# 23skdu/longbow

Measured on AMD Instinct MI355X. Metric: k-NN queries/sec (batch=1024, k=100), 1Mx768 f32, higher is better.
Workload: dtype f32; 1 GPU; 1Mx768 float32 cosine, batch=1024 queries, k=100, brute-force; dim=768, batch=1024, k=100, metric=cosine, global_rows=1000000, candidate_mode=LB_CAND_F32_MFMA (strict; the library default is AUTO: auto_path leg)

## Files before the change

### longbow_amd/_lib.py

```python
import ctypes as C
import os

_HERE = os.path.dirname(os.path.abspath(__file__))
SO_PATH = os.environ.get("LB_GPU_SO") or os.path.join(_HERE, "liblongbow_gpu.so")

LB_OK = 0
STATUS = {0: "ok", 1: "invalid argument", 2: "index is closed", 3: "GPU not available",
          4: "HIP runtime error", 5: "out of device memory", 6: "unsupported configuration",
          7: "internal error", 8: "context canceled", 9: "context deadline exceeded"}


class LongbowGPUError(RuntimeError):
    def __init__(self, code, msg=""):
        self.code = code
        super().__init__(f"longbow_gpu: {STATUS.get(code, 'error')} (code {code}){': ' + msg if msg else ''}")


class GPUNotAvailable(LongbowGPUError):
    """internal/gpu/stub.go:10 ErrGPUNotAvailable"""


class Canceled(LongbowGPUError):
    """context.Canceled: the call's Cancel fired (internal/store/adaptive_index.go:182 returns ctx.Err())"""

# ... 229 lines not shown
    ("lb_gpu_ivfpq_dims", _i, [_vp]),
    ("lb_gpu_ivfpq_m", _i, [_vp]),
    ("lb_gpu_ivfpq_order", _i, [_vp]),
    ("lb_gpu_ivfpq_nlist", _i, [_vp]),
    ("lb_gpu_ivfpq_ntotal", _i64, [_vp]),
    ("lb_gpu_ivfpq_hbm_bytes", _i64, [_vp]),
    ("lb_gpu_ivfpq_get_centroids", _i, [_vp, _vp]),
    ("lb_gpu_ivfpq_reserve", _i, [_vp, _i64]),
    ("lb_gpu_ivfpq_add", _i, [_vp, _i64, _vp, _vp]),
    ("lb_gpu_ivfpq_add_device", _i, [_vp, _i64, _vp, _vp]),
    ("lb_gpu_ivfpq_get_codes", _i, [_vp, _i64, _i64, _vp]),
    ("lb_gpu_ivfpq_list_sizes", _i, [_vp, _vp]),
    ("lb_gpu_ivfpq_assignments", _i, [_vp, _i64, _i64, _vp]),
    ("lb_gpu_ivfpq_search", _i, [_vp, _i64, _vp, _i, _i, _vp, _vp]),
    ("lb_gpu_ivfpq_search_ctx", _i, [_vp, _i64, _vp, _i, _i, _vp, _vp, _vp]),
    ("lb_gpu_ivfpq_search_device_ctx", _i, [_vp, _i64, _vp, _i, _i, _vp, _vp, _vp, _vp]),
    ("lb_gpu_ivfpq_set_filter", _i, [_vp, _vp, _i64]),
    ("lb_gpu_ivfpq_filter_int64", _i, [_vp, _vp, _i64, _i64, _i, _vp, _i64, _i]),
    ("lb_gpu_ivfpq_filter_float32", _i, [_vp, _vp, _i64, C.c_float, _i, _vp, _i64, _i]),
    ("lb_gpu_ivfpq_nvisible", _i64, [_vp]),
    ("lb_gpu_ivfpq_last_search_stats", _i, [_vp, C.POINTER(C.c_int64)]),
    ("lb_gpu_ivfpq_set_profiling", _i, [_vp, _i]),
    ("lb_gpu_ivfpq_last_timing", _i, [_vp, _vp]),
    ("lb_gpu_ivfpq_last_build_timing", _i, [_vp, _vp]),
    ("lb_gpu_ivfpq_remove", _i, [_vp, _i64, _vp, C.POINTER(C.c_int64)]),
    ("lb_gpu_ivfpq_remove_device", _i, [_vp, _i64, _vp, C.POINTER(C.c_int64)]),
    ("lb_gpu_ivfpq_remove_rows", _i, [_vp, _i64, _vp, C.POINTER(C.c_int64)]),
    ("lb_gpu_ivfpq_nlive", _i64, [_vp]),
    ("lb_gpu_ivfpq_ndeleted", _i64, [_vp]),
    ("lb_gpu_ivfpq_compact", _i, [_vp, _vp, _i64]),
    ("lb_gpu_ivfsq8_new", _vp, [_i, _i, _vp, _vp, _i, _i, _vp, _ip]),
    ("lb_gpu_ivfsq8_free", None, [_vp]),
    ("lb_gpu_ivfsq8_last_error", C.c_char_p, [_vp]),
    ("lb_gpu_ivfsq8_dims", _i, [_vp]),
    ("lb_gpu_ivfsq8_order", _i, [_vp]),
    ("lb_gpu_ivfsq8_nlist", _i, [_vp]),
    ("lb_gpu_ivfsq8_ntotal", _i64, [_vp]),
    ("lb_gpu_ivfsq8_hbm_bytes", _i64, [_vp]),
    ("lb_gpu_ivfsq8_get_bounds", _i, [_vp, _vp, _vp]),
    ("lb_gpu_ivfsq8_get_centroids", _i, [_vp, _vp]),
    ("lb_gpu_ivfsq8_reserve", _i, [_vp, _i64]),
    ("lb_gpu_ivfsq8_add", _i, [_vp, _i64, _vp, _vp]),
    ("lb_gpu_ivfsq8_add_device", _i, [_vp, _i64, _vp, _vp]),
    ("lb_gpu_ivfsq8_get_codes", _i, [_vp, _i64, _i64, _vp]),
    ("lb_gpu_ivfsq8_list_sizes", _i, [_vp, _vp]),
    ("lb_gpu_ivfsq8_assignments", _i, [_vp, _i64, _i64, _vp]),
    ("lb_gpu_ivfsq8_search", _i, [_vp, _i64, _vp, _i, _i, _vp, _vp]),
    ("lb_gpu_ivfsq8_search_ctx", _i, [_vp, _i64, _vp, _i, _i, _vp, _vp, _vp]),
    ("lb_gpu_ivfsq8_search_device_ctx", _i, [_vp, _i64, _vp, _i, _i, _vp, _vp, _vp, _vp]),
    ("lb_gpu_ivfsq8_set_filter", _i, [_vp, _vp, _i64]),
    ("lb_gpu_ivfsq8_filter_int64", _i, [_vp, _vp, _i64, _i64, _i, _vp, _i64, _i]),
    ("lb_gpu_ivfsq8_filter_float32", _i, [_vp, _vp, _i64, C.c_float, _i, _vp, _i64, _i]),
    ("lb_gpu_ivfsq8_nvisible", _i64, [_vp]),
    ("lb_gpu_ivfsq8_last_search_stats", _i, [_vp, C.POINTER(C.c_int64)]),
    ("lb_gpu_ivfsq8_set_profiling", _i, [_vp, _i]),
    ("lb_gpu_ivfsq8_last_timing", _i, [_vp, _vp]),
    ("lb_gpu_ivfsq8_last_build_timing", _i, [_vp, _vp]),
    ("lb_gpu_ivfsq8_remove", _i, [_vp, _i64, _vp, C.POINTER(C.c_int64)]),
    ("lb_gpu_ivfsq8_remove_device", _i, [_vp, _i64, _vp, C.POINTER(C.c_int64)]),
    ("lb_gpu_ivfsq8_remove_rows", _i, [_vp, _i64, _vp, C.POINTER(C.c_int64)]),
    ("lb_gpu_ivfsq8_nlive", _i64, [_vp]),
    ("lb_gpu_ivfsq8_ndeleted", _i64, [_vp]),
    ("lb_gpu_ivfsq8_compact", _i, [_vp, _vp, _i64]),
    ("lb_gpu_ivfbq_new", _vp, [_i, _i, _i, _i, _vp, _ip]),
    ("lb_gpu_ivfbq_free", None, [_vp]),
    ("lb_gpu_ivfbq_last_error", C.c_char_p, [_vp]),
    ("lb_gpu_ivfbq_dims", _i, [_vp]),
    ("lb_gpu_ivfbq_words", _i, [_vp]),
    ("lb_gpu_ivfbq_order", _i, [_vp]),
    ("lb_gpu_ivfbq_nlist", _i, [_vp]),
    ("lb_gpu_ivfbq_ntotal", _i64, [_vp]),
    ("lb_gpu_ivfbq_hbm_bytes", _i64, [_vp]),
    ("lb_gpu_ivfbq_get_centroids", _i, [_vp, _vp]),
    ("lb_gpu_ivfbq_reserve", _i, [_vp, _i64]),
    ("lb_gpu_ivfbq_add", _i, [_vp, _i64, _vp, _vp]),
    ("lb_gpu_ivfbq_add_device", _i, [_vp, _i64, _vp, _vp]),
    ("lb_gpu_ivfbq_get_codes", _i, [_vp, _i64, _i64, _vp]),
    ("lb_gpu_ivfbq_list_sizes", _i, [_vp, _vp]),
    ("lb_gpu_ivfbq_assignments", _i, [_vp, _i64, _i64, _vp]),
    ("lb_gpu_ivfbq_search", _i, [_vp, _i64, _vp, _i, _i, _vp, _vp]),
    ("lb_gpu_ivfbq_search_ctx", _i, [_vp, _i64, _vp, _i, _i, _vp, _vp, _vp]),
    ("lb_gpu_ivfbq_search_device_ctx", _i, [_vp, _i64, _vp, _i, _i, _vp, _vp, _vp, _vp]),
    ("lb_gpu_ivfbq_set_filter", _i, [_vp, _vp, _i64]),
    ("lb_gpu_ivfbq_filter_int64", _i, [_vp, _vp, _i64, _i64, _i, _vp, _i64, _i]),
    ("lb_gpu_ivfbq_filter_float32", _i, [_vp, _vp, _i64, C.c_float, _i, _vp, _i64, _i]),
    ("lb_gpu_ivfbq_nvisible", _i64, [_vp]),
    ("lb_gpu_ivfbq_last_search_stats", _i, [_vp, C.POINTER(C.c_int64)]),
    ("lb_gpu_ivfbq_set_profiling", _i, [_vp, _i]),
    ("lb_gpu_ivfbq_last_timing", _i, [_vp, _vp]),
    ("lb_gpu_ivfbq_last_build_timing", _i, [_vp, _vp]),
    ("lb_gpu_merge_topk_device", _i, [_i, _i, _i64, _i, _vp, _vp, _vp, _vp, _vp]),
    ("lb_gpu_merge_topk_packed_device", _i, [_i, _i, _i64, _i, _vp, _vp, _vp, _vp]),
    ("lb_gpu_rrf_fuse_device", _i, [_i, _i64, _i, _vp, _i, _vp, _i, _i, _vp, _vp, _vp]),
    ("lb_gpu_rrf_fuse", _i, [_i, _i64, _i, _vp, _i, _vp, _i, _i, _vp, _vp]),
    ("lb_gpu_fill_uniform_device", _i, [_i, _vp, _i64, _u64, _i64, _vp]),
    ("lb_gpu_fill_codes_device", _i, [_i, _vp, _i64, _u64, _i64, _vp]),
    ("lb_gpu_fill_uniform_rows_device", _i, [_i, _vp, _vp, _i64, _i, _u64, _vp]),
    ("lb_gpu_shader_clock_mhz", C.c_double, [_i, _i]),
    ("lb_flight_datasets_new", _vp, []),
    ("lb_flight_datasets_free", None, [_vp]),
    ("lb_flight_datasets_put", _i, [_vp, C.c_char_p, _vp]),
    ("lb_flight_vector_search_exchange", _i, [_vp, _vp, _sz, C.POINTER(_vp), C.POINTER(_sz), C.c_char_p, _sz]),
    ("lb_flight_encode_results", _i, [_vp, _vp, _i64, C.POINTER(_vp), C.POINTER(_sz)]),
    ("lb_flight_free_buffer", None, [_vp]),
    ("lb_flight_index_add_ipc", _i, [_vp, _vp, _sz, C.POINTER(_i64), C.c_char_p, _sz]),
    ("lb_gpu_comm_init_all", _vp, [_i, _vp, _ip]),
    ("lb_gpu_comm_get_unique_id", _i, [_vp]),
    ("lb_gpu_comm_init_rank", _vp, [_i, _i, _i, _vp, _ip]),
    ("lb_gpu_comm_init_host", _vp, [_i, _i, _i, _vp, _vp, _ip]),
    ("lb_gpu_comm_free", None, [_vp]),
    ("lb_gpu_comm_prepare", _i, [_vp, _i64, _i]),
    ("lb_gpu_comm_nranks", _i, [_vp]),
    ("lb_gpu_comm_rank", _i, [_vp]),
    ("lb_gpu_comm_last_error", C.c_char_p, [_vp]),
    ("lb_gpu_comm_search_device", _i, [_vp, _vp, _i64, _vp, _i, _vp, _vp, _vp]),
    ("lb_gpu_comm_search_all", _i, [_vp, _vp, _i64, _vp, _i, _vp, _vp]),
    ("lb_gpu_index_set_profiling", _i, [_vp, _i]),
    ("lb_gpu_index_last_timing", _i, [_vp, _vp, _vp]),
]


def _bind(path, extra=()):
    if not os.path.exists(path):
        raise RuntimeError(
            f"{path} is missing: build it with `python -m longbow_amd.build{' --diag' if extra else ''}` "
            "(hipcc --offload-arch=gfx950).  There is no CPU fallback.")
    lib = C.CDLL(path)
    for name, res, args in list(SIGNATURES) + list(extra):
        fn = getattr(lib, name)
        fn.restype = res
        fn.argtypes = args
    return lib


def load():
    global _lib
    if _lib is None:
        _lib = _bind(SO_PATH)
    return _lib


DIAG_SO_PATH = os.path.join(_HERE, "liblongbow_gpu_diag.so")
DIAG_SIGNATURES = [
    ("lb_debug_set_sample_tau", None, [_i]),
    ("lb_debug_vmm_fail_next", None, [_i]),
    ("lb_debug_fused_fail_next", None, [_i]),
    ("lb_debug_tin_withhold_next", None, [_i]),
    ("lb_debug_search_fail_next", None, [_i]),
    ("lb_debug_set_add_register_min", None, [C.c_longlong]),
    ("lb_debug_sample_plan", None, [C.c_longlong, _i, C.c_uint, C.c_uint, C.POINTER(C.c_longlong)]),
    ("lb_debug_cand_geometry", None, [_i, C.POINTER(C.c_int), C.POINTER(C.c_uint)]),
    ("lb_debug_last_wide_rows", _i, []),
    ("lb_debug_set_wide256_min_tiles", None, [_i]),
    ("lb_debug_set_compact_round_rows", None, [C.c_longlong]),
]
_diag = None


def load_diag():
    global _diag
    if _diag is None:
        _diag = _bind(DIAG_SO_PATH, DIAG_SIGNATURES)
    return _diag


def require_gpu(device=0):
    lib = load()
    n = lib.lb_gpu_device_count()
    if n <= 0 or device >= n:
        raise GPUNotAvailable(3, f"{n} HIP device(s) visible, device {device} requested")
    return lib


def check(rc, handle=None, lib=None, prefix=None):
    if rc == LB_OK:
        return
    msg = ""
    if handle:
        lib = lib or load()
        raw = getattr(lib, prefix + "_last_error" if prefix else "lb_gpu_last_error")(handle)
        msg = raw.decode() if raw else ""
    if rc == 3:
        raise GPUNotAvailable(rc, msg)
    if rc == 8:
        raise Canceled(rc, msg)
    if rc == 9:
        raise DeadlineExceeded(rc, msg)
    raise LongbowGPUError(rc, msg)
```

### longbow_amd/csrc/kernels_gemm.hip

```cpp
#include "lb_admit.h"

#include <atomic>
#include <cstdlib>

namespace lb {

constexpr int BM = 128;
constexpr int BN = 128;
constexpr int BK = 32;
constexpr int GEMM_THREADS = 256;

struct GemmArgs {
    const float *X;
    const float *norm2;
    const float *rnorm;
    int64_t row_begin, row_end;
    int D;
    const float *Q;
    int nq;
    const uint8_t *mask;
    const uint32_t *rowmap;
    CandState cs;
    int n_row_tiles, n_q_tiles;
    int boot;
};

__device__ __forceinline__ int swz_off(int row, int chunk)
{
    return row * BK + ((chunk ^ ((row >> 1) & 7)) << 2);
}

template <int MODE>
__device__ __forceinline__ f32x4 load_chunk(const float *base, int64_t row, int D, int k)
{
    f32x4 v = {0.f, 0.f, 0.f, 0.f};
    const float *p = base + row * (int64_t)D + k;
    if (MODE == 2) {
        v = *reinterpret_cast<const f32x4 *>(p);
    } else if (MODE == 1) {
        if (k < D) v = *reinterpret_cast<const f32x4 *>(p);
    } else {
        if (k + 0 < D) v.x = p[0];
        if (k + 1 < D) v.y = p[1];
        if (k + 2 < D) v.z = p[2];
        if (k + 3 < D) v.w = p[3];
    }
    return v;
}

template <int METRIC, int ALIGNED>
__global__ __launch_bounds__(GEMM_THREADS, 2) void gemm_filter_kernel(GemmArgs a)
{
    constexpr bool GLDS = ALIGNED == 2;
    const int b = blockIdx.x;
    const int xcd = b & 7;
    const int in_xcd = b >> 3;
    const int qt = in_xcd % a.n_q_tiles;
    const int rt = (in_xcd / a.n_q_tiles) * 8 + xcd;
    if (rt >= a.n_row_tiles) return;

    __shared__ __attribute__((aligned(16))) float lds_all[2 * 2 * BM * BK + BM + BM + BM / 4];
    float(*lds)[2][BM * BK] = reinterpret_cast<float(*)[2][BM * BK]>(lds_all);
    float *s_aux = lds_all + 2 * 2 * BM * BK;
    uint32_t *s_rowid = reinterpret_cast<uint32_t *>(s_aux + BM);
    uint8_t *s_vis = reinterpret_cast<uint8_t *>(s_rowid + BM);

    const int tid = threadIdx.x;
    const int lane = tid & 63;
    const int wave = tid >> 6;
    const int wr = wave >> 1, wc = wave & 1;
    const int l31 = lane & 31, h = lane >> 5;

    const int64_t row0 = a.row_begin + (int64_t)rt * BM;
    const int q0 = qt * BN;
    const int64_t last_row = a.row_end - 1;
    const int last_q = a.nq - 1;

    auto corpus_row = [&](int64_t pos) -> int64_t {
        if (pos > last_row) pos = last_row;
        return a.rowmap ? (int64_t)a.rowmap[pos] : pos;
    };
    const int64_t side_ri = corpus_row(row0 + (tid & (BM - 1)));

    int st_row[4], st_ch[4];
    int64_t st_xrow[4];
    int st_qrow[4];
#pragma unroll
    for (int i = 0; i < 4; i++) {
        int c = tid + GEMM_THREADS * i;
        st_row[i] = c >> 3;
        st_ch[i] = c & 7;
        st_xrow[i] = corpus_row(row0 + st_row[i]);
        int qr = q0 + st_row[i];
        st_qrow[i] = qr < last_q ? qr : last_q;
    }

    f32x16 acc[2][2];
#pragma unroll
    for (int i = 0; i < 2; i++)
#pragma unroll
        for (int j = 0; j < 2; j++)
#pragma unroll
            for (int r = 0; r < 16; r++) acc[i][j][r] = 0.f;

    const int nk = (a.D + BK - 1) / BK;
    f32x4 ra[4], rb[4];

    const float *gsrcA[4], *gsrcB[4];
    if (GLDS) {
#pragma unroll
        for (int i = 0; i < 4; i++) {
            const int j = wave * 4 + i;
            const int row = j * 8 + (lane >> 3);
            const int c = (lane & 7) ^ ((row >> 1) & 7);
            const int64_t xr = corpus_row(row0 + row);
            int qr = q0 + row;
            if (qr > last_q) qr = last_q;
            gsrcA[i] = a.X + xr * (int64_t)a.D + 4 * c;
            gsrcB[i] = a.Q + (int64_t)qr * a.D + 4 * c;
        }
    }
    const int wave_u = __builtin_amdgcn_readfirstlane(wave);
    auto glds_piece = [&](int p, int stage, int k0) {
        const int i = p >> 1;
        const int j = wave_u * 4 + i;
        if ((p & 1) == 0)
            __builtin_amdgcn_global_load_lds(
                (const __attribute__((address_space(1))) void *)(gsrcA[i] + k0),
                (__attribute__((address_space(3))) void *)(&lds[stage][0][j * 8 * BK]), 16, 0,
                2);
        else
            __builtin_amdgcn_global_load_lds(
                (const __attribute__((address_space(1))) void *)(gsrcB[i] + k0),
                (__attribute__((address_space(3))) void *)(&lds[stage][1][j * 8 * BK]), 16, 0, 0);
    };
    auto glds_stage = [&](int stage, int k0) {
#pragma unroll
        for (int p = 0; p < 8; p++) glds_piece(p, stage, k0);
    };
    if (GLDS) glds_stage(0, 0);
    const float aux_r = side_aux<METRIC>(a.norm2, a.rnorm, side_ri);
    uint8_t side_vis = 1;
    if (a.mask) side_vis = a.mask[side_ri];
    uint64_t tau_raw[2];
#pragma unroll
    for (int tn = 0; tn < 2; tn++) {
        const int qj = q0 + wc * 64 + tn * 32 + l31;
        tau_raw[tn] = lane_tau(a.cs.tau, qj, a.nq, a.boot);
    }
    if (tid < BM) {
        s_aux[tid] = aux_r;
        s_vis[tid] = (row0 + tid <= last_row && side_vis) ? (uint8_t)1 : (uint8_t)0;
        s_rowid[tid] = (uint32_t)side_ri;
    }
    float tau_key[2];
    uint32_t tau_row[2];
#pragma unroll
    for (int tn = 0; tn < 2; tn++) {
// ... 102 lines not shown
            const float *As = lds[cur][0];
            const float *Bs = lds[cur][1];
            f32x4 fa[2][2], fb[2][2];
#pragma unroll
            for (int t = 0; t < 2; t++) {
                fa[0][t] = *reinterpret_cast<const f32x4 *>(&As[swz_off(wr * 64 + t * 32 + l31, h)]);
                fb[0][t] = *reinterpret_cast<const f32x4 *>(&Bs[swz_off(wc * 64 + t * 32 + l31, h)]);
            }
#pragma unroll
            for (int s = 0; s < 4; s++) {
                const int cb = s & 1, nb = cb ^ 1;
                if (s < 3) {
                    const int ch = 2 * (s + 1) + h;
#pragma unroll
                    for (int t = 0; t < 2; t++) {
                        fa[nb][t] = *reinterpret_cast<const f32x4 *>(&As[swz_off(wr * 64 + t * 32 + l31, ch)]);
                        fb[nb][t] = *reinterpret_cast<const f32x4 *>(&Bs[swz_off(wc * 64 + t * 32 + l31, ch)]);
                    }
                }
#pragma unroll
                for (int e = 0; e < 4; e++)
#pragma unroll
                    for (int tm = 0; tm < 2; tm++)
#pragma unroll
                        for (int tn = 0; tn < 2; tn++)
                            acc[tm][tn] = __builtin_amdgcn_mfma_f32_32x32x2f32(fa[cb][tm][e], fb[cb][tn][e],
                                                                              acc[tm][tn], 0, 0, 0);
                if (s == 1 && has_next) {
                    const int nxt = cur ^ 1;
#pragma unroll
                    for (int i = 0; i < 4; i++) {
                        *reinterpret_cast<f32x4 *>(&lds[nxt][0][swz_off(st_row[i], st_ch[i])]) = ra[i];
                        *reinterpret_cast<f32x4 *>(&lds[nxt][1][swz_off(st_row[i], st_ch[i])]) = rb[i];
                    }
                }
            }
            __syncthreads();
        }
    }

    float aux[2][4][4];
    uint32_t rid[2][4][4];
    uint32_t vbits = 0;
#pragma unroll
    for (int tm = 0; tm < 2; tm++)
#pragma unroll
        for (int g = 0; g < 4; g++)
            vbits |= tile_rows4(s_aux, s_rowid, s_vis, wr * 64 + tm * 32 + 8 * g + 4 * h, aux[tm][g], rid[tm][g]) << (tm * 16 + g * 4);
#pragma unroll
    for (int tn = 0; tn < 2; tn++) {
        const int qj = q0 + wc * 64 + tn * 32 + l31;
        const bool qok = qj < a.nq;
        uint64_t *list = a.cs.lists + (size_t)(qok ? qj : 0) * a.cs.cap;
        if (a.boot) {
            if (qok) {
#pragma unroll
                for (int tm = 0; tm < 2; tm++)
#pragma unroll
                    for (int g = 0; g < 4; g++) {
                        const int64_t rbase = row0 + wr * 64 + tm * 32 + 8 * g + 4 * h;
                        uint64_t ent[4];
#pragma unroll
                        for (int e = 0; e < 4; e++)
                            ent[e] = ((vbits >> (tm * 16 + g * 4 + e)) & 1u) ? pack_entry(cand_key<METRIC>(acc[tm][tn][4 * g + e], aux[tm][g][e]), rid[tm][g][e]) : kEntryMax;
                        uint64_t *dst = list + (rbase - a.row_begin);
                        if (rbase + 3 < a.row_end) {
                            typedef unsigned long long u64x2 __attribute__((ext_vector_type(2)));
                            u64x2 v0 = {ent[0], ent[1]}, v1 = {ent[2], ent[3]};
                            *reinterpret_cast<u64x2 *>(dst) = v0;
                            *reinterpret_cast<u64x2 *>(dst + 2) = v1;
                        } else {
#pragma unroll
                            for (int e = 0; e < 4; e++)
                                if (rbase + e < a.row_end) dst[e] = ent[e];
                        }
                    }
            }
            continue;
        }
        uint32_t bits = 0;
#pragma unroll
        for (int tm = 0; tm < 2; tm++)
#pragma unroll
            for (int g = 0; g < 4; g++)
#pragma unroll
                for (int e = 0; e < 4; e++)
                    bits |= admit_exact(cand_key<METRIC>(acc[tm][tn][4 * g + e], aux[tm][g][e]), rid[tm][g][e], tau_key[tn], tau_row[tn]) << (tm * 16 + g * 4 + e);
        bits &= vbits;
        if (bits) {
            uint32_t pos = atomicAdd(&a.cs.cnt[qj], (uint32_t)__builtin_popcount(bits));
#pragma unroll
            for (int tm = 0; tm < 2; tm++)
#pragma unroll
                for (int g = 0; g < 4; g++)
#pragma unroll
                    for (int e = 0; e < 4; e++)
                        if (bits & (1u << (tm * 16 + g * 4 + e))) {
                            const uint32_t ri = rid[tm][g][e];
                            if (pos < a.cs.cap) list[pos] = pack_entry(cand_key<METRIC>(acc[tm][tn][4 * g + e], aux[tm][g][e]), ri);
                            pos++;
                        }
        }
    }
}

constexpr int WBM = 256;
constexpr int WBK = 16;
constexpr int WNST = 3;
constexpr int W_STAGE_F = (WBM + BN) * WBK;
constexpr int W_NI = 6;

__device__ __forceinline__ int wswz(int row, int chunk) { return row * WBK + ((chunk ^ ((row >> 2) & 3)) << 2); }

template <bool NT>
__device__ __forceinline__ void wide_dma16(const void *gsrc, uint32_t lds_addr)
{
    uint32_t save;
    if (NT)
        asm volatile("s_mov_b32 %0, m0\n\ts_mov_b32 m0, %2\n\ts_nop 0\n\tglobal_load_lds_dwordx4 %1, off nt\n\ts_mov_b32 m0, %0"
                     : "=&s"(save) : "v"(gsrc), "s"(lds_addr) : "memory");
    else
        asm volatile("s_mov_b32 %0, m0\n\ts_mov_b32 m0, %2\n\ts_nop 0\n\tglobal_load_lds_dwordx4 %1, off\n\ts_mov_b32 m0, %0"
                     : "=&s"(save) : "v"(gsrc), "s"(lds_addr) : "memory");
}
template <int VM, int LGKM>
__device__ __forceinline__ void wide_wait()
{
    __builtin_amdgcn_s_waitcnt((VM & 15) | (7 << 4) | (LGKM << 8) | ((VM >> 4) << 14));
    asm volatile("" ::: "memory");
}
constexpr bool kWide256CorpusNT = false;

template <int VM>
__device__ __forceinline__ void wide_step_barrier()
{
    wide_wait<VM, 0>();
    __builtin_amdgcn_s_barrier();
    asm volatile("" ::: "memory");
}

struct WideFrag {
    f32x4 a[4], b[2];
};
template <int FROM, int TO>
__device__ __forceinline__ void wide_mfma(f32x16 (&acc)[4][2], const WideFrag &f)
{
#pragma unroll
    for (int i = FROM; i < TO; i++) {
        const int e = i >> 3, tm = (i >> 1) & 3, tn = i & 1;
        acc[tm][tn] = __builtin_amdgcn_mfma_f32_32x32x2f32(f.a[tm][e], f.b[tn][e], acc[tm][tn], 0, 0, 0);
    }
}

template <int METRIC>
__global__ __launch_bounds__(GEMM_THREADS, 2) void gemm_filter_wide256_kernel(GemmArgs a)
{
    const int b = blockIdx.x;
    const int xcd = b & 7;
    const int in_xcd = b >> 3;
    const int qt = in_xcd % a.n_q_tiles;
    const int rt = (in_xcd / a.n_q_tiles) * 8 + xcd;
    if (rt >= a.n_row_tiles) return;

    __shared__ __attribute__((aligned(16))) float lds_all[WNST * W_STAGE_F + WBM + WBM + WBM / 4];
    float *ring = lds_all;
    float *s_aux = ring + WNST * W_STAGE_F;
    uint32_t *s_rowid = reinterpret_cast<uint32_t *>(s_aux + WBM);
    uint8_t *s_vis = reinterpret_cast<uint8_t *>(s_rowid + WBM);
    const uint32_t ring_base = (uint32_t)(uintptr_t)(__attribute__((address_space(3))) float *)ring;

    const int tid = threadIdx.x;
    const int lane = tid & 63;
    const int wave = __builtin_amdgcn_readfirstlane(tid >> 6);
    const int wr = wave >> 1, wc = wave & 1;
    const int l31 = lane & 31, h = lane >> 5;

    const int64_t row0 = a.row_begin + (int64_t)rt * WBM;
    const int q0 = qt * BN;
    const int64_t last_row = a.row_end - 1;
    const int last_q = a.nq - 1;

    auto corpus_row = [&](int64_t pos) -> int64_t {
        if (pos > last_row) pos = last_row;
        return a.rowmap ? (int64_t)a.rowmap[pos] : pos;
    };
    const int64_t side_ri = corpus_row(row0 + tid);

    const float *srcA[4], *srcB[2];
#pragma unroll
    for (int i = 0; i < 4; i++) {
        const int row = wave * 64 + i * 16 + (lane >> 2);
        const int c = (lane & 3) ^ ((row >> 2) & 3);
        srcA[i] = a.X + corpus_row(row0 + row) * (int64_t)a.D + 4 * c;
    }
#pragma unroll
    for (int i = 0; i < 2; i++) {
        const int row = wave * 32 + i * 16 + (lane >> 2);
        const int c = (lane & 3) ^ ((row >> 2) & 3);
        int qr = q0 + row;
        if (qr > last_q) qr = last_q;
        srcB[i] = a.Q + (int64_t)qr * a.D + 4 * c;
    }
    auto piece = [&](int p, int slot, int k0) {
        const uint32_t A = ring_base + (uint32_t)slot * (W_STAGE_F * 4);
        if (p < 4)
            wide_dma16<kWide256CorpusNT>(srcA[p] + k0, A + (uint32_t)((wave * 64 + p * 16) * WBK * 4));
        else
            wide_dma16<false>(srcB[p - 4] + k0, A + (uint32_t)(WBM * WBK * 4 + (wave * 32 + (p - 4) * 16) * WBK * 4));
    };
    auto issue = [&](int slot, int k0) {
#pragma unroll
        for (int p = 0; p < W_NI; p++) piece(p, slot, k0);
    };

    f32x16 acc[4][2];
#pragma unroll
    for (int i = 0; i < 4; i++)
#pragma unroll
        for (int j = 0; j < 2; j++)
#pragma unroll
            for (int r = 0; r < 16; r++) acc[i][j][r] = 0.f;

    const int nk = a.D / WBK;
    issue(0, 0);
    issue(1, WBK);
    if (nk > 2) issue(2, 2 * WBK);
    const float aux_r = side_aux<METRIC>(a.norm2, a.rnorm, side_ri);
    uint8_t side_vis = 1;
    if (a.mask) side_vis = a.mask[side_ri];
    uint64_t tau_raw[2];
#pragma unroll
    for (int tn = 0; tn < 2; tn++) tau_raw[tn] = lane_tau(a.cs.tau, q0 + wc * 64 + tn * 32 + l31, a.nq, false);
    s_aux[tid] = aux_r;
    s_vis[tid] = (row0 + tid <= last_row && side_vis) ? (uint8_t)1 : (uint8_t)0;
    s_rowid[tid] = (uint32_t)side_ri;
    float tau_key[2];
    uint32_t tau_row[2];
#pragma unroll
    for (int tn = 0; tn < 2; tn++) {
        tau_key[tn] = tau_key_of(tau_raw[tn]);
        tau_row[tn] = entry_row(tau_raw[tn]);
    }
    wide_wait<0, 0>();
    __syncthreads();

    WideFrag F0, F1;
    auto ldfrag = [&](WideFrag &f, int slot, int s) {
        const float *As = ring + slot * W_STAGE_F;
        const float *Bs = As + WBM * WBK;
        const int ch = 2 * s + h;
#pragma unroll
        for (int t = 0; t < 4; t++) f.a[t] = *reinterpret_cast<const f32x4 *>(&As[wswz(wr * 128 + t * 32 + l31, ch)]);
#pragma unroll
        for (int t = 0; t < 2; t++) f.b[t] = *reinterpret_cast<const f32x4 *>(&Bs[wswz(wc * 64 + t * 32 + l31, ch)]);
    };
    auto sub0 = [&](int slot) {
        wide_mfma<0, 2>(acc, F0);
        __builtin_amdgcn_sched_barrier(0);
        ldfrag(F1, slot, 1);
        __builtin_amdgcn_sched_barrier(0);
        wide_mfma<2, 32>(acc, F0);
        __builtin_amdgcn_sched_barrier(0);
    };
    auto sub1 = [&](int next_slot) {
        wide_mfma<0, 2>(acc, F1);
        __builtin_amdgcn_sched_barrier(0);
        ldfrag(F0, next_slot, 0);
        __builtin_amdgcn_sched_barrier(0);
        wide_mfma<2, 32>(acc, F1);
        __builtin_amdgcn_sched_barrier(0);
    };
    auto sub1_dma = [&](int next_slot, int dma_slot, int k0) {
        wide_mfma<0, 2>(acc, F1);
        __builtin_amdgcn_sched_barrier(0);
        ldfrag(F0, next_slot, 0);
        __builtin_amdgcn_sched_barrier(0);
        wide_mfma<2, 8>(acc, F1);
        __builtin_amdgcn_sched_barrier(0);
#define LB_W256_PIECE(P)                                \
    piece(P, dma_slot, k0);                             \
    __builtin_amdgcn_sched_barrier(0);                  \
    wide_mfma<8 + 4 * (P), 12 + 4 * (P)>(acc, F1);      \
    __builtin_amdgcn_sched_barrier(0);
        LB_W256_PIECE(0) LB_W256_PIECE(1) LB_W256_PIECE(2) LB_W256_PIECE(3) LB_W256_PIECE(4) LB_W256_PIECE(5)
#undef LB_W256_PIECE
    };
    ldfrag(F0, 0, 0);
    int slot = 0;
    int j = 0;
    for (; j + 3 < nk; j++) {
        const int next = slot == WNST - 1 ? 0 : slot + 1;
        sub0(slot);
        wide_step_barrier<W_NI>();
        sub1_dma(next, slot, (j + 3) * WBK);
        slot = next;
    }
    if (j + 2 < nk) {
        const int next = slot == WNST - 1 ? 0 : slot + 1;
        sub0(slot);
        wide_step_barrier<W_NI>();
        sub1(next);
        slot = next;
    }
    {
        const int next = slot == WNST - 1 ? 0 : slot + 1;
        sub0(slot);
        wide_step_barrier<0>();
        sub1(next);
        slot = next;
    }
    sub0(slot);
    wide_mfma<0, 32>(acc, F1);
    __builtin_amdgcn_sched_barrier(0);

    uint64_t bits[2] = {0ull, 0ull};
#pragma unroll
    for (int tm = 0; tm < 4; tm++) {
        float aux[4][4];
        uint32_t rid[4][4];
        uint32_t vb = 0;
#pragma unroll
        for (int g = 0; g < 4; g++) vb |= tile_rows4(s_aux, s_rowid, s_vis, wr * 128 + tm * 32 + 8 * g + 4 * h, aux[g], rid[g]) << (g * 4);
#pragma unroll
        for (int tn = 0; tn < 2; tn++) {
            uint32_t bb = 0;
#pragma unroll
            for (int g = 0; g < 4; g++)
#pragma unroll
                for (int e = 0; e < 4; e++) {
                    bb |= admit_exact(cand_key<METRIC>(acc[tm][tn][4 * g + e], aux[g][e]), rid[g][e], tau_key[tn], tau_row[tn]) << (g * 4 + e);
                }
            bits[tn] |= (uint64_t)(bb & vb) << (tm * 16);
        }
        __builtin_amdgcn_sched_barrier(0);
    }
    int lr2 = wr * 128 + 4 * h;
    asm volatile("" : "+v"(lr2), "+v"(bits[0]), "+v"(bits[1]));
#pragma unroll
    for (int tn = 0; tn < 2; tn++) {
        if (!bits[tn]) continue;
        const int qj = q0 + wc * 64 + tn * 32 + l31;
        uint64_t *list = a.cs.lists + (size_t)qj * a.cs.cap;
        uint32_t pos = atomicAdd(&a.cs.cnt[qj], (uint32_t)__builtin_popcountll(bits[tn]));
#pragma unroll
        for (int tm = 0; tm < 4; tm++) {
            const uint32_t bb = (uint32_t)(bits[tn] >> (tm * 16)) & 0xffffu;
            if (!bb) continue;
#pragma unroll
            for (int g = 0; g < 4; g++) {
                const uint32_t nib = (bb >> (g * 4)) & 15u;
                if (!nib) continue;
                float aux[4];
                uint32_t rid[4];
                (void)tile_rows4(s_aux, s_rowid, s_vis, lr2 + tm * 32 + 8 * g, aux, rid);
#pragma unroll
                for (int e = 0; e < 4; e++)
                    if (nib & (1u << e)) {
                        if (pos < a.cs.cap) list[pos] = pack_entry(cand_key<METRIC>(acc[tm][tn][4 * g + e], aux[e]), rid[e]);
                        pos++;
                    }
            }
        }
    }
}

__global__ __launch_bounds__(256) void split_bf16_kernel(const float *src, float *dst, int64_t n8)
{
    for (int64_t i = (int64_t)blockIdx.x * blockDim.x + threadIdx.x; i < n8; i += (int64_t)gridDim.x * blockDim.x) {
        bf16x8 hi, lo;
        split_bf16x8(*reinterpret_cast<const f32x4 *>(src + i * 8), *reinterpret_cast<const f32x4 *>(src + i * 8 + 4), hi, lo);
        const int64_t grp = i >> 1;
        const int kb = (int)(i & 1);
        char *g = reinterpret_cast<char *>(dst) + grp * 64;
        *reinterpret_cast<bf16x8 *>(g + kb * 16) = hi;
        *reinterpret_cast<bf16x8 *>(g + 32 + kb * 16) = lo;
    }
}

void launch_split_bf16(const float *src, float *dst, int64_t rows, int D, hipStream_t s)
{
    const int64_t n8 = rows * (int64_t)D / 8;
    if (n8 <= 0) return;
    int64_t blocks = (n8 + 255) / 256;
    if (blocks > 16384) blocks = 16384;
    hipLaunchKernelGGL(split_bf16_kernel, dim3((unsigned)blocks), dim3(256), 0, s, src, dst, n8);
}

constexpr int kWide256MinTiles = 6144;
#ifdef LB_DIAG
static std::atomic<int> g_wide256_min_tiles{kWide256MinTiles};
static std::atomic<int> g_last_wide_rows{0};
#endif

void launch_gemm_filter(int metric, const float *X, const float *norm2, const float *rnorm,
                        int64_t row_begin, int64_t row_end, int D, const float *Q, int nq,
                        const uint8_t *mask, const uint32_t *rowmap, CandState cs, bool boot, hipStream_t s)
{
    if (row_end <= row_begin || nq <= 0) return;
    GemmArgs a;
    a.rowmap = rowmap;
    a.boot = boot ? 1 : 0;
    a.X = X; a.norm2 = norm2; a.rnorm = rnorm;
    a.row_begin = row_begin; a.row_end = row_end; a.D = D;
    a.Q = Q; a.nq = nq; a.mask = mask; a.cs = cs;
    a.n_q_tiles = (nq + BN - 1) / BN;
    const bool aligned = (D % 4 == 0) && ((reinterpret_cast<uintptr_t>(X) & 15) == 0) &&
                         ((reinterpret_cast<uintptr_t>(Q) & 15) == 0);
    const int mode = !aligned ? 0 : (D % BK == 0 ? 2 : 1);
#ifdef LB_DIAG
    const int wide256_min = g_wide256_min_tiles.load(std::memory_order_relaxed);
#else
    const int wide256_min = kWide256MinTiles;
#endif
    const int64_t tiles256 = (row_end - row_begin + WBM - 1) / WBM;
    const bool wide256 = !boot && mode == 2 && tiles256 * a.n_q_tiles >= wide256_min;
#ifdef LB_DIAG
    if (!boot) g_last_wide_rows.store(wide256 ? WBM : BM, std::memory_order_relaxed);
#endif
    a.n_row_tiles = wide256 ? (int)tiles256 : (int)((row_end - row_begin + BM - 1) / BM);
    const int groups = (a.n_row_tiles + 7) / 8;
    dim3 grid((unsigned)(groups * 8 * a.n_q_tiles));
#define LB_GEMM(M, AL) hipLaunchKernelGGL((gemm_filter_kernel<M, AL>), grid, dim3(GEMM_THREADS), 0, s, a)
#define LB_GEMM_M(M)                 \
    do {                             \
        if (wide256) hipLaunchKernelGGL((gemm_filter_wide256_kernel<M>), grid, dim3(GEMM_THREADS), 0, s, a); \
        else if (mode == 2) LB_GEMM(M, 2); \
        else if (mode == 1) LB_GEMM(M, 1); \
        else LB_GEMM(M, 0);           \
    } while (0)
    if (metric == METRIC_L2) LB_GEMM_M(METRIC_L2);
    else if (metric == METRIC_COS) LB_GEMM_M(METRIC_COS);
    else LB_GEMM_M(METRIC_DOT);
#undef LB_GEMM_M
#undef LB_GEMM
}

}

#ifdef LB_DIAG
extern "C" {
int lb_debug_last_wide_rows(void) { return lb::g_last_wide_rows.load(); }
void lb_debug_set_wide256_min_tiles(int v)
{
    lb::g_wide256_min_tiles.store(v < 0 ? lb::kWide256MinTiles : v);
    lb::g_last_wide_rows.store(0);
}
}
#endif
```

Before: 89640 queries/s.

## Make wide256 GEMM filter persistent and prefetch next tile during epilogue

Turns the wide256 candidate-filter GEMM kernel into a persistent kernel with a grid of about 2×CU blocks. Each block walks its tile list with a per-XCD stride. While the tail MFMAs of the current tile run, the first K-stages of the next tile are prefetched, and side data (norms, mask, row ids) is double-buffered in LDS. The intent is to hide per-tile prologue latency and launch/tail effects. In exchange it raises LDS use, adds register pressure, and makes the tail harder to schedule.

```diff
diff --git a/longbow_amd/_lib.py b/longbow_amd/_lib.py
--- a/longbow_amd/_lib.py
+++ b/longbow_amd/_lib.py
@@ -405,6 +405,7 @@
     ("lb_debug_cand_geometry", None, [_i, C.POINTER(C.c_int), C.POINTER(C.c_uint)]),
     ("lb_debug_last_wide_rows", _i, []),
     ("lb_debug_set_wide256_min_tiles", None, [_i]),
+    ("lb_debug_set_wide_walk_groups", None, [_i]),
     ("lb_debug_set_compact_round_rows", None, [C.c_longlong]),
 ]
 _diag = None
diff --git a/longbow_amd/csrc/kernels_gemm.hip b/longbow_amd/csrc/kernels_gemm.hip
--- a/longbow_amd/csrc/kernels_gemm.hip
+++ b/longbow_amd/csrc/kernels_gemm.hip
@@ -4,6 +4,11 @@
 #include <cstdlib>
 
 namespace lb {
+#ifdef LB_X_NOPF
+#define LB_X_PF false
+#else
+#define LB_X_PF true
+#endif
 
 constexpr int BM = 128;
 constexpr int BN = 128;
@@ -412,21 +417,39 @@
     }
 }
 
+template <int FROM, int TO>
+__device__ __forceinline__ void wide_tail_mfma(f32x16 (&acc)[4][2], const WideFrag &f0, const WideFrag &f1)
+{
+    constexpr int N0 = 30;
+    wide_mfma<(FROM < N0 ? FROM : N0) + 2, (TO < N0 ? TO : N0) + 2>(acc, f0);
+    wide_mfma<(FROM > N0 ? FROM : N0) - N0, (TO > N0 ? TO : N0) - N0>(acc, f1);
+}
+
 template <int METRIC>
 __global__ __launch_bounds__(GEMM_THREADS, 2) void gemm_filter_wide256_kernel(GemmArgs a)
 {
     const int b = blockIdx.x;
     const int xcd = b & 7;
-    const int in_xcd = b >> 3;
-    const int qt = in_xcd % a.n_q_tiles;
-    const int rt = (in_xcd / a.n_q_tiles) * 8 + xcd;
-    if (rt >= a.n_row_tiles) return;
-
-    __shared__ __attribute__((aligned(16))) float lds_all[WNST * W_STAGE_F + WBM + WBM + WBM / 4];
+    const int wstep = (int)(gridDim.x >> 3);
+    const int n_list = xcd < a.n_row_tiles ? ((a.n_row_tiles - xcd + 7) >> 3) * a.n_q_tiles : 0;
+    int in_xcd = b >> 3;
+    if (in_xcd >= n_list) return;
+#ifdef LB_X_PHASE_HALF
+    if (b >= (int)(gridDim.x >> 1)) for (int i = 0; i < 26; i++) __builtin_amdgcn_s_sleep(127);
+#endif
+#ifdef LB_X_PHASE_ODD
+    if ((b >> 3) & 1) for (int i = 0; i < 26; i++) __builtin_amdgcn_s_sleep(127);
+#endif
+    const bool fast_ok = !a.rowmap && wstep % a.n_q_tiles == 0;
+    const int fast_rt = (wstep / a.n_q_tiles) * 8;
+    int qt = in_xcd % a.n_q_tiles;
+    int rt = (in_xcd / a.n_q_tiles) * 8 + xcd;
+
+    __shared__ __attribute__((aligned(16))) float lds_all[WNST * W_STAGE_F + 2 * (WBM + WBM + WBM / 4)];
     float *ring = lds_all;
     float *s_aux = ring + WNST * W_STAGE_F;
-    uint32_t *s_rowid = reinterpret_cast<uint32_t *>(s_aux + WBM);
-    uint8_t *s_vis = reinterpret_cast<uint8_t *>(s_rowid + WBM);
+    uint32_t *s_rowid = reinterpret_cast<uint32_t *>(s_aux + 2 * WBM);
+    uint8_t *s_vis = reinterpret_cast<uint8_t *>(s_rowid + 2 * WBM);
     const uint32_t ring_base = (uint32_t)(uintptr_t)(__attribute__((address_space(3))) float *)ring;
 
     const int tid = threadIdx.x;
@@ -435,8 +458,8 @@
     const int wr = wave >> 1, wc = wave & 1;
     const int l31 = lane & 31, h = lane >> 5;
 
-    const int64_t row0 = a.row_begin + (int64_t)rt * WBM;
-    const int q0 = qt * BN;
+    int64_t row0 = a.row_begin + (int64_t)rt * WBM;
+    int q0 = qt * BN;
     const int64_t last_row = a.row_end - 1;
     const int last_q = a.nq - 1;
 
@@ -444,23 +467,43 @@
         if (pos > last_row) pos = last_row;
         return a.rowmap ? (int64_t)a.rowmap[pos] : pos;
     };
-    const int64_t side_ri = corpus_row(row0 + tid);
 
     const float *srcA[4], *srcB[2];
-#pragma unroll
-    for (int i = 0; i < 4; i++) {
-        const int row = wave * 64 + i * 16 + (lane >> 2);
-        const int c = (lane & 3) ^ ((row >> 2) & 3);
-        srcA[i] = a.X + corpus_row(row0 + row) * (int64_t)a.D + 4 * c;
-    }
-#pragma unroll
-    for (int i = 0; i < 2; i++) {
-        const int row = wave * 32 + i * 16 + (lane >> 2);
-        const int c = (lane & 3) ^ ((row >> 2) & 3);
-        int qr = q0 + row;
-        if (qr > last_q) qr = last_q;
-        srcB[i] = a.Q + (int64_t)qr * a.D + 4 * c;
-    }
+    auto set_sources = [&](int64_t r0, int qq0) {
+        int ln = lane;
+        asm volatile("" : "+v"(ln));
+#pragma unroll
+        for (int i = 0; i < 4; i++) {
+            const int row = wave * 64 + i * 16 + (ln >> 2);
+            const int c = (ln & 3) ^ ((row >> 2) & 3);
+            srcA[i] = a.X + corpus_row(r0 + row) * (int64_t)a.D + 4 * c;
+        }
+#pragma unroll
+        for (int i = 0; i < 2; i++) {
+            const int row = wave * 32 + i * 16 + (ln >> 2);
+            const int c = (ln & 3) ^ ((row >> 2) & 3);
+            int qr = qq0 + row;
+            if (qr > last_q) qr = last_q;
+            srcB[i] = a.Q + (int64_t)qr * a.D + 4 * c;
+        }
+    };
+    set_sources(row0, q0);
+    float side_a;
+    uint32_t side_r;
+    uint8_t side_v;
+    auto side_load = [&](int64_t r0) {
+        const int64_t ri = corpus_row(r0 + tid);
+        side_a = side_aux<METRIC>(a.norm2, a.rnorm, ri);
+        uint8_t vis = 1;
+        if (a.mask) vis = a.mask[ri];
+        side_v = (r0 + tid <= last_row && vis) ? (uint8_t)1 : (uint8_t)0;
+        side_r = (uint32_t)ri;
+    };
+    auto side_store = [&](int buf) {
+        s_aux[buf * WBM + tid] = side_a;
+        s_vis[buf * WBM + tid] = side_v;
+        s_rowid[buf * WBM + tid] = side_r;
+    };
     auto piece = [&](int p, int slot, int k0) {
         const uint32_t A = ring_base + (uint32_t)slot * (W_STAGE_F * 4);
         if (p < 4)
@@ -474,35 +517,27 @@
     };
 
     f32x16 acc[4][2];
-#pragma unroll
-    for (int i = 0; i < 4; i++)
-#pragma unroll
-        for (int j = 0; j < 2; j++)
-#pragma unroll
-            for (int r = 0; r < 16; r++) acc[i][j][r] = 0.f;
 
     const int nk = a.D / WBK;
     issue(0, 0);
     issue(1, WBK);
     if (nk > 2) issue(2, 2 * WBK);
-    const float aux_r = side_aux<METRIC>(a.norm2, a.rnorm, side_ri);
-    uint8_t side_vis = 1;
-    if (a.mask) side_vis = a.mask[side_ri];
-    uint64_t tau_raw[2];
-#pragma unroll
-    for (int tn = 0; tn < 2; tn++) tau_raw[tn] = lane_tau(a.cs.tau, q0 + wc * 64 + tn * 32 + l31, a.nq, false);
-    s_aux[tid] = aux_r;
-    s_vis[tid] = (row0 + tid <= last_row && side_vis) ? (uint8_t)1 : (uint8_t)0;
-    s_rowid[tid] = (uint32_t)side_ri;
     float tau_key[2];
     uint32_t tau_row[2];
-#pragma unroll
-    for (int tn = 0; tn < 2; tn++) {
-        tau_key[tn] = tau_key_of(tau_raw[tn]);
-        tau_row[tn] = entry_row(tau_raw[tn]);
-    }
-    wide_wait<0, 0>();
-    __syncthreads();
+    auto load_tau = [&](int qq0) {
+        uint64_t tau_raw[2];
+#pragma unroll
+        for (int tn = 0; tn < 2; tn++) tau_raw[tn] = lane_tau(a.cs.tau, qq0 + wc * 64 + tn * 32 + l31, a.nq, false);
+#pragma unroll
+        for (int tn = 0; tn < 2; tn++) {
+            tau_key[tn] = tau_key_of(tau_raw[tn]);
+            tau_row[tn] = entry_row(tau_raw[tn]);
+        }
+    };
+    side_load(row0);
+    load_tau(q0);
+    side_store(0);
+    int cur = 0;
 
     WideFrag F0, F1;
     auto ldfrag = [&](WideFrag &f, int slot, int s) {
@@ -545,82 +580,139 @@
         LB_W256_PIECE(0) LB_W256_PIECE(1) LB_W256_PIECE(2) LB_W256_PIECE(3) LB_W256_PIECE(4) LB_W256_PIECE(5)
 #undef LB_W256_PIECE
     };
-    ldfrag(F0, 0, 0);
-    int slot = 0;
-    int j = 0;
-    for (; j + 3 < nk; j++) {
-        const int next = slot == WNST - 1 ? 0 : slot + 1;
-        sub0(slot);
-        wide_step_barrier<W_NI>();
-        sub1_dma(next, slot, (j + 3) * WBK);
-        slot = next;
-    }
-    if (j + 2 < nk) {
-        const int next = slot == WNST - 1 ? 0 : slot + 1;
-        sub0(slot);
-        wide_step_barrier<W_NI>();
-        sub1(next);
-        slot = next;
-    }
-    {
-        const int next = slot == WNST - 1 ? 0 : slot + 1;
-        sub0(slot);
-        wide_step_barrier<0>();
-        sub1(next);
-        slot = next;
-    }
-    sub0(slot);
-    wide_mfma<0, 32>(acc, F1);
-    __builtin_amdgcn_sched_barrier(0);
-
-    uint64_t bits[2] = {0ull, 0ull};
-#pragma unroll
-    for (int tm = 0; tm < 4; tm++) {
-        float aux[4][4];
-        uint32_t rid[4][4];
-        uint32_t vb = 0;
-#pragma unroll
-        for (int g = 0; g < 4; g++) vb |= tile_rows4(s_aux, s_rowid, s_vis, wr * 128 + tm * 32 + 8 * g + 4 * h, aux[g], rid[g]) << (g * 4);
+    for (;;) {
+#pragma unroll
+        for (int i = 0; i < 4; i++)
+#pragma unroll
+            for (int j = 0; j < 2; j++)
+#pragma unroll
+                for (int r = 0; r < 16; r++) acc[i][j][r] = 0.f;
+        wide_wait<0, 0>();
+        __syncthreads();
+
+        const int next_in = in_xcd + wstep;
+        const bool has_next = next_in < n_list;
+        const int next_qt = fast_ok ? qt : next_in % a.n_q_tiles;
+        const int next_rt = fast_ok ? rt + fast_rt : (next_in / a.n_q_tiles) * 8 + xcd;
+        const int64_t next_row0 = a.row_begin + (int64_t)next_rt * WBM;
+        const int next_q0 = next_qt * BN;
+
+        ldfrag(F0, 0, 0);
+        int slot = 0;
+        int j = 0;
+        for (; j + 3 < nk; j++) {
+            const int next = slot == WNST - 1 ? 0 : slot + 1;
+            sub0(slot);
+            wide_step_barrier<W_NI>();
+            sub1_dma(next, slot, (j + 3) * WBK);
+            slot = next;
+        }
+        if (j + 2 < nk) {
+            const int next = slot == WNST - 1 ? 0 : slot + 1;
+            sub0(slot);
+            wide_step_barrier<W_NI>();
+            sub1(next);
+            slot = next;
+        }
+        {
+            const int next = slot == WNST - 1 ? 0 : slot + 1;
+            sub0(slot);
+            wide_step_barrier<0>();
+            sub1(next);
+            slot = next;
+        }
+        wide_mfma<0, 2>(acc, F0);
+        __builtin_amdgcn_sched_barrier(0);
+        ldfrag(F1, slot, 1);
+        __builtin_amdgcn_sched_barrier(0);
+        if (has_next) {
+            wide_step_barrier<0>();
+            if (fast_ok && next_row0 + WBM <= a.row_end) {
+                const int64_t adv = (int64_t)fast_rt * WBM * a.D;
+#pragma unroll
+                for (int i = 0; i < 4; i++) srcA[i] += adv;
+            } else {
+                set_sources(next_row0, next_q0);
+            }
+        }
+        const bool next_third = has_next && nk > 2;
+        __builtin_amdgcn_sched_barrier(0);
+        wide_tail_mfma<0, 8>(acc, F0, F1);
+        __builtin_amdgcn_sched_barrier(0);
+#define LB_W256_NEXT(P)                                                                            \
+        if (LB_X_PF && ((P) < 2 * W_NI ? has_next : next_third)) piece((P) % W_NI, (P) / W_NI, ((P) / W_NI) * WBK); \
+        __builtin_amdgcn_sched_barrier(0);                                                             \
+        wide_tail_mfma<8 + 3 * (P), 11 + 3 * (P)>(acc, F0, F1);                                        \
+        __builtin_amdgcn_sched_barrier(0);
+        LB_W256_NEXT(0) LB_W256_NEXT(1) LB_W256_NEXT(2) LB_W256_NEXT(3) LB_W256_NEXT(4) LB_W256_NEXT(5)
+        LB_W256_NEXT(6) LB_W256_NEXT(7) LB_W256_NEXT(8) LB_W256_NEXT(9) LB_W256_NEXT(10) LB_W256_NEXT(11)
+        LB_W256_NEXT(12) LB_W256_NEXT(13) LB_W256_NEXT(14) LB_W256_NEXT(15) LB_W256_NEXT(16) LB_W256_NEXT(17)
+#undef LB_W256_NEXT
+        if (has_next) side_load(next_row0);
+        __builtin_amdgcn_sched_barrier(0);
+        const float *c_aux = s_aux + cur * WBM;
+        const uint32_t *c_rowid = s_rowid + cur * WBM;
+        const uint8_t *c_vis = s_vis + cur * WBM;
+
+        uint64_t bits[2] = {0ull, 0ull};
+#pragma unroll
+        for (int tm = 0; tm < 4; tm++) {
+            float aux[4][4];
+            uint32_t rid[4][4];
+            uint32_t vb = 0;
+#pragma unroll
+            for (int g = 0; g < 4; g++) vb |= tile_rows4(c_aux, c_rowid, c_vis, wr * 128 + tm * 32 + 8 * g + 4 * h, aux[g], rid[g]) << (g * 4);
+#pragma unroll
+            for (int tn = 0; tn < 2; tn++) {
+                uint32_t bb = 0;
+#pragma unroll
+                for (int g = 0; g < 4; g++)
+#pragma unroll
+                    for (int e = 0; e < 4; e++) {
+                        bb |= admit_exact(cand_key<METRIC>(acc[tm][tn][4 * g + e], aux[g][e]), rid[g][e], tau_key[tn], tau_row[tn]) << (g * 4 + e);
+                    }
+                bits[tn] |= (uint64_t)(bb & vb) << (tm * 16);
+            }
+            __builtin_amdgcn_sched_barrier(0);
+        }
+        int lr2 = wr * 128 + 4 * h;
+        asm volatile("" : "+v"(lr2), "+v"(bits[0]), "+v"(bits[1]));
 #pragma unroll
         for (int tn = 0; tn < 2; tn++) {
-            uint32_t bb = 0;
-#pragma unroll
-            for (int g = 0; g < 4; g++)
-#pragma unroll
-                for (int e = 0; e < 4; e++) {
-                    bb |= admit_exact(cand_key<METRIC>(acc[tm][tn][4 * g + e], aux[g][e]), rid[g][e], tau_key[tn], tau_row[tn]) << (g * 4 + e);
+            if (!bits[tn]) continue;
+            const int qj = q0 + wc * 64 + tn * 32 + l31;
+            uint64_t *list = a.cs.lists + (size_t)qj * a.cs.cap;
+            uint32_t pos = atomicAdd(&a.cs.cnt[qj], (uint32_t)__builtin_popcountll(bits[tn]));
+#pragma unroll
+            for (int tm = 0; tm < 4; tm++) {
+                const uint32_t bb = (uint32_t)(bits[tn] >> (tm * 16)) & 0xffffu;
+                if (!bb) continue;
+#pragma unroll
+                for (int g = 0; g < 4; g++) {
+                    const uint32_t nib = (bb >> (g * 4)) & 15u;
+                    if (!nib) continue;
+                    float aux[4];
+                    uint32_t rid[4];
+                    (void)tile_rows4(c_aux, c_rowid, c_vis, lr2 + tm * 32 + 8 * g, aux, rid);
+#pragma unroll
+                    for (int e = 0; e < 4; e++)
+                        if (nib & (1u << e)) {
+                            if (pos < a.cs.cap) list[pos] = pack_entry(cand_key<METRIC>(acc[tm][tn][4 * g + e], aux[e]), rid[e]);
+                            pos++;
+                        }
                 }
-            bits[tn] |= (uint64_t)(bb & vb) << (tm * 16);
-        }
-        __builtin_amdgcn_sched_barrier(0);
-    }
-    int lr2 = wr * 128 + 4 * h;
-    asm volatile("" : "+v"(lr2), "+v"(bits[0]), "+v"(bits[1]));
-#pragma unroll
-    for (int tn = 0; tn < 2; tn++) {
-        if (!bits[tn]) continue;
-        const int qj = q0 + wc * 64 + tn * 32 + l31;
-        uint64_t *list = a.cs.lists + (size_t)qj * a.cs.cap;
-        uint32_t pos = atomicAdd(&a.cs.cnt[qj], (uint32_t)__builtin_popcountll(bits[tn]));
-#pragma unroll
-        for (int tm = 0; tm < 4; tm++) {
-            const uint32_t bb = (uint32_t)(bits[tn] >> (tm * 16)) & 0xffffu;
-            if (!bb) continue;
-#pragma unroll
-            for (int g = 0; g < 4; g++) {
-                const uint32_t nib = (bb >> (g * 4)) & 15u;
-                if (!nib) continue;
-                float aux[4];
-                uint32_t rid[4];
-                (void)tile_rows4(s_aux, s_rowid, s_vis, lr2 + tm * 32 + 8 * g, aux, rid);
-#pragma unroll
-                for (int e = 0; e < 4; e++)
-                    if (nib & (1u << e)) {
-                        if (pos < a.cs.cap) list[pos] = pack_entry(cand_key<METRIC>(acc[tm][tn][4 * g + e], aux[e]), rid[e]);
-                        pos++;
-                    }
-            }
-        }
+            }
+        }
+        if (!has_next) break;
+        if (!LB_X_PF) { issue(0, 0); issue(1, WBK); if (nk > 2) issue(2, 2 * WBK); }
+        cur ^= 1;
+        side_store(cur);
+        if (next_q0 != q0) load_tau(next_q0);
+        in_xcd = next_in;
+        qt = next_qt;
+        rt = next_rt;
+        row0 = next_row0;
+        q0 = next_q0;
     }
 }
 
@@ -650,7 +742,35 @@
 #ifdef LB_DIAG
 static std::atomic<int> g_wide256_min_tiles{kWide256MinTiles};
 static std::atomic<int> g_last_wide_rows{0};
-#endif
+static std::atomic<int> g_wide_walk_groups{-1};
+#endif
+
+static int wide_walk_groups(int64_t tiles)
+{
+    constexpr int kMaxDev = 64;
+    static std::atomic<int> cus_of[kMaxDev];
+    int dev = 0, cus = 0;
+    (void)hipGetDevice(&dev);
+    if (dev >= 0 && dev < kMaxDev) cus = cus_of[dev].load(std::memory_order_relaxed);
+    if (cus == 0) {
+        if (hipDeviceGetAttribute(&cus, hipDeviceAttributeMultiprocessorCount, dev) != hipSuccess || cus <= 0) cus = -1;
+        if (dev >= 0 && dev < kMaxDev) cus_of[dev].store(cus, std::memory_order_relaxed);
+    }
+    int64_t g = cus > 0 ? 2 * (int64_t)cus : tiles;
+#ifdef LB_DIAG
+    const int forced = g_wide_walk_groups.load(std::memory_order_relaxed);
+    if (forced >= 0) g = forced;
+#endif
+#ifdef LB_X_G_TILES
+    g = tiles;
+#endif
+#ifdef LB_X_DIV
+    g = (tiles / LB_X_DIV) & ~(int64_t)63;
+#endif
+    if (g > tiles) g = tiles;
+    g &= ~(int64_t)7;
+    return g < 8 ? 8 : (int)g;
+}
 
 void launch_gemm_filter(int metric, const float *X, const float *norm2, const float *rnorm,
                         int64_t row_begin, int64_t row_end, int D, const float *Q, int nq,
@@ -680,10 +800,11 @@
     a.n_row_tiles = wide256 ? (int)tiles256 : (int)((row_end - row_begin + BM - 1) / BM);
     const int groups = (a.n_row_tiles + 7) / 8;
     dim3 grid((unsigned)(groups * 8 * a.n_q_tiles));
+    const dim3 walk_grid(wide256 ? (unsigned)wide_walk_groups(tiles256 * a.n_q_tiles) : 1u);
 #define LB_GEMM(M, AL) hipLaunchKernelGGL((gemm_filter_kernel<M, AL>), grid, dim3(GEMM_THREADS), 0, s, a)
 #define LB_GEMM_M(M)                 \
     do {                             \
-        if (wide256) hipLaunchKernelGGL((gemm_filter_wide256_kernel<M>), grid, dim3(GEMM_THREADS), 0, s, a); \
+        if (wide256) hipLaunchKernelGGL((gemm_filter_wide256_kernel<M>), walk_grid, dim3(GEMM_THREADS), 0, s, a); \
         else if (mode == 2) LB_GEMM(M, 2); \
         else if (mode == 1) LB_GEMM(M, 1); \
         else LB_GEMM(M, 0);           \
@@ -705,5 +826,6 @@
     lb::g_wide256_min_tiles.store(v < 0 ? lb::kWide256MinTiles : v);
     lb::g_last_wide_rows.store(0);
 }
-}
-#endif
+void lb_debug_set_wide_walk_groups(int v) { lb::g_wide_walk_groups.store(v < 0 ? -1 : v); }
+}
+#endif
```

Measured after the change: 88660 queries/s. 1.1% lower.
